# HumaticsLAB/SEAM-Match-RCNN

Measured on NVIDIA B200. Metric: pair_scores_per_sec, higher is better.
Workload: dtype f32 (fp16-operand tcgen05 pass nominates candidates, every result re-scored in f32)

## Files before the change

seam-match-rcnn_b200/csrc/score_exact.cuh:

```cuda
#pragma once
#include <type_traits>
#include <climits>
#include <cstdint>
#include <cuda_fp16.h>
#include "exchange.cuh"
#include "fold.cuh"
#include "score_tc.cuh"
#include "sm100_ptx.cuh"
#include "warp_sort.cuh"

namespace seam {
namespace exact {

constexpr float FP16_MAX = 65504.f;
constexpr float EPS_COEFF = 9.9e-4f;
constexpr float TAG_REL_ERR = 8e-6f;

__device__ __forceinline__ float softmax1(float l0, float l1) {
  const float m = fmaxf(l0, l1);
  const float e0 = expf(l0 - m), e1 = expf(l1 - m);
  return e1 / (e0 + e1);
}

struct Slice {
// ... 43 lines not shown
  l1 = ptx::warp_sum_b(p1) + b1;
}

__global__ void __launch_bounds__(256) prep_gallery_kernel(const float* __restrict__ g, int G,
                                                           const float* __restrict__ fold, __half* __restrict__ g16,
                                                           float* __restrict__ cg, float* __restrict__ gstat) {
  const int warp = threadIdx.x >> 5, lane = threadIdx.x & 31;
  const int j = blockIdx.x * 8 + warp;
  if (j >= G) return;
  const Slice x = load_slice(g + (size_t)j * 256, lane);
  const Slice dw = load_slice(fold + Fold::DW, lane);
  const float xs[8] = {x.lo.x, x.lo.y, x.lo.z, x.lo.w, x.hi.x, x.hi.y, x.hi.z, x.hi.w};
  const float ds[8] = {dw.lo.x, dw.lo.y, dw.lo.z, dw.lo.w, dw.hi.x, dw.hi.y, dw.hi.z, dw.hi.w};
  float c = 0.f, n2 = 0.f, amax = 0.f;
  __half h[8];
#pragma unroll
  for (int e = 0; e < 8; ++e) {
    c = fmaf(ds[e], xs[e] * xs[e], c);
    n2 = fmaf(xs[e], xs[e], n2);
    amax = fmaxf(amax, fabsf(xs[e]));
    h[e] = __float2half_rn(xs[e]);
  }
  __half* dst = g16 + (size_t)j * 256;
  *reinterpret_cast<uint2*>(dst + 4 * lane) = *reinterpret_cast<const uint2*>(&h[0]);
  *reinterpret_cast<uint2*>(dst + 128 + 4 * lane) = *reinterpret_cast<const uint2*>(&h[4]);
  c = ptx::warp_sum(c);
  n2 = ptx::warp_sum(n2);
  amax = ptx::warp_max(amax);
  if (lane == 0) {
    cg[j] = c;
    atomicMax(reinterpret_cast<unsigned int*>(gstat), __float_as_uint(sqrtf(n2)));
    if (!(amax < FP16_MAX)) atomicMax(reinterpret_cast<unsigned int*>(gstat + 1), __float_as_uint(1.f));
  }
}

__global__ void __launch_bounds__(256) prep_queries_kernel(const float* q, int Q,
                                                           const float* __restrict__ fold, __half* __restrict__ a16,
                                                           float* __restrict__ rq, float* __restrict__ anorm,
                                                           uint32_t* __restrict__ thr_global,
                                                           uint32_t* __restrict__ rowflag,
                                                           int32_t* __restrict__ counters,
                                                           int32_t* __restrict__ xdone, const int x_on,
                                                           const xchg::Exchange xc) {
  const int warp = threadIdx.x >> 5, lane = threadIdx.x & 31;
  const int i = blockIdx.x * 8 + warp;
  if (x_on) {
    const uint32_t step = xchg::current_step(xc);
    xchg::wait_all(xc, xchg::KIND_Q, step);
    q = xc.q_all[xc.rank] + (size_t)(step & 1u) * xc.Q * 256;
  }
  if (blockIdx.x == 0 && threadIdx.x == 0) {
    counters[0] = 0;
    counters[1] = 0;
  }
  if (i >= Q) return;
  const Slice x = load_slice(q + (size_t)i * 256, lane);
  const Slice dw = load_slice(fold + Fold::DW, lane);
  const float xs[8] = {x.lo.x, x.lo.y, x.lo.z, x.lo.w, x.hi.x, x.hi.y, x.hi.z, x.hi.w};
  const float ds[8] = {dw.lo.x, dw.lo.y, dw.lo.z, dw.lo.w, dw.hi.x, dw.hi.y, dw.hi.z, dw.hi.w};
  float r = 0.f, n2 = 0.f, amax = 0.f;
  __half h[8];
#pragma unroll
  for (int e = 0; e < 8; ++e) {
    const float a = -2.f * ds[e] * xs[e];
    r = fmaf(ds[e], xs[e] * xs[e], r);
    n2 = fmaf(a, a, n2);
    amax = fmaxf(amax, fabsf(a));
    h[e] = __float2half_rn(a);
  }
  __half* dst = a16 + (size_t)i * 256;
  *reinterpret_cast<uint2*>(dst + 4 * lane) = *reinterpret_cast<const uint2*>(&h[0]);
  *reinterpret_cast<uint2*>(dst + 128 + 4 * lane) = *reinterpret_cast<const uint2*>(&h[4]);
  r = ptx::warp_sum(r);
  n2 = ptx::warp_sum(n2);
  amax = ptx::warp_max(amax);
  if (lane == 0) {
    rq[i] = r;
    anorm[i] = sqrtf(n2);
    thr_global[i] = ptx::float_to_ordered(-INFINITY);
    rowflag[i] = 0;
    if (xdone) xdone[i] = 0;
    if (!(amax < FP16_MAX)) atomicExch(counters + 1, 1);
  }
}

struct RescoreParams {
  const float* q;
  const float* g;
  const float* fold;
  const uint2* rowbuf;
  const uint32_t* rowcnt;
  const uint32_t* rowflag;
  const uint32_t* thr_global;
  const float* gmax;
  const float* rq;
  const float* anorm;
  const float* gstat;
  int Q, G, nlists, CAP, k, index_offset;
  float* out_score;
  float* out_margin;
  int32_t* out_idx;
  int32_t* counters;
  int32_t* fallback_rows;
  int x_on;
  xchg::Exchange x;
  score::TilePlan plan;
};

struct TopkDest {
  float* score;
  float* margin;
  int32_t* idx;
};
__device__ __forceinline__ TopkDest topk_dest(int x_on, const xchg::Exchange& x, uint32_t step, int qi, int k,
                                              float* out_score, float* out_margin, int32_t* out_idx) {
  TopkDest d;
  if (!x_on) {
    const size_t o = (size_t)qi * k;
    d.score = out_score + o;
    d.margin = out_margin + o;
    d.idx = out_idx + o;
  } else {
    const int ow = xchg::owner_of(x, qi);
    const size_t o = ((((size_t)(step & 1u) * x.world + x.rank) * x.own_max) + (size_t)(qi - x.q_lo[ow])) * k;
    d.score = nullptr;
    d.margin = x.list_margin[ow] + o;
    d.idx = x.list_idx[ow] + o;
  }
  return d;
}

constexpr int RS_SUBL = 4;
constexpr int RESCORE_WBUF = 160;

__device__ __forceinline__ void rescore_merge32(const uint2* wb, int begin, int end, float& cv, uint32_t& cidx,
                                                int lane) {
  float v = -INFINITY;
  uint32_t id = 0xffffffffu;
  if (begin + lane < end) {
    const uint2 e = wb[begin + lane];
    v = __uint_as_float(e.x);
    id = e.y;
  }
  const float worst = __shfl_sync(ptx::FULL_MASK, cv, 31);
  if (!(v > worst)) {
    v = -INFINITY;
    id = 0xffffffffu;
  }
  if (!__any_sync(ptx::FULL_MASK, v > -INFINITY)) return;
  wsort::sort32<false>(v, id, lane);
  if (v > cv) {
    cv = v;
    cidx = id;
  }
  wsort::merge32<true>(cv, cidx, lane);
}

__global__ void __launch_bounds__(256) rescore_kernel(const RescoreParams p) {
  __shared__ uint2 wbuf[8][RESCORE_WBUF];
  __shared__ uint4 qbuf[8][64];
  __shared__ uint32_t qcol[8][64];
  const int warp = threadIdx.x >> 5, lane = threadIdx.x & 31;
  const int qi = blockIdx.x * 8 + warp;
  if (qi >= p.Q) return;
  const uint32_t xstep = p.x_on ? xchg::current_step(p.x) : 0u;
  const float* qbase = p.x_on ? p.x.q_all[p.x.rank] + (size_t)(xstep & 1u) * p.x.Q * 256 : p.q;
  const bool overflow = p.counters[1] != 0 || p.gstat[1] != 0.f;
  bool certified = !overflow && p.rowflag[qi] == 0;
  const float tau = ptx::ordered_to_float(p.thr_global[qi]);
  const int nl_valid = min(p.nlists, 4 * score::pieces_of_row(p.plan, qi));
  float cv = -INFINITY;
  uint32_t cidx = 0xffffffffu;
  uint2* wb = wbuf[warp];
  int fill = 0;
  float cut = tau;
  bool cut_strict = false;
  float cut_lo = tau > -INFINITY ? nextafterf(tau, -INFINITY) : -INFINITY;
  {
    const int nval = nl_valid * 16;
    const float* gmp = p.gmax + (size_t)qi * p.nlists * 16;
    auto start_cut = [&](auto nk_tag) {
      constexpr int NK = decltype(nk_tag)::value;
      uint32_t key[NK];
#pragma unroll
      for (int u = 0; u < NK; ++u) {
        const int i = lane + 32 * u;
        key[u] = i < nval ? ptx::float_to_ordered(gmp[i]) : 0u;
      }
      uint32_t lmax = key[0];
#pragma unroll
      for (int j = 1; j < NK; ++j) lmax = max(lmax, key[j]);
      const uint32_t hi = __reduce_max_sync(ptx::FULL_MASK, lmax);
      const uint32_t lo = __reduce_min_sync(ptx::FULL_MASK, lmax);
      uint32_t K = lo;
      if (hi != lo) {
        const int b0 = 31 - __clz(hi ^ lo);
        K = hi & ~((2u << b0) - 1u);
        for (int b = b0; b >= 0 && b > b0 - 8; --b) {
          const uint32_t T = K | (1u << b);
          uint32_t c = 0;
#pragma unroll
          for (int j = 0; j < NK; ++j)
            asm("{\n.reg .pred p;\nsetp.ge.u32 p, %1, %2;\n@p add.u32 %0, %0, 1;\n}\n" : "+r"(c) : "r"(key[j]), "r"(T));
          if (__reduce_add_sync(ptx::FULL_MASK, c) >= 32u) K = T;
        }
      }
      const float tt = ptx::ordered_to_float(K);
      if (K != 0 && tt > cut) {
        cut = tt;
        cut_lo = nextafterf(tt, -INFINITY);
      }
    };
    if (nval <= 128) start_cut(std::integral_constant<int, 4>{});
    else if (nval <= 256) start_cut(std::integral_constant<int, 8>{});
  }
  const int capq = p.CAP / 2;
  const uint4* rowq = reinterpret_cast<const uint4*>(p.rowbuf) + (size_t)qi * p.nlists * capq;
  uint4* qb = qbuf[warp];
  uint32_t* qc = qcol[warp];
  int qfill = 0;
  auto expand = [&](int start, int count) {
    uint4 rec = make_uint4(0u, 0u, 0u, 0u);
    uint32_t col = 0;
    const bool have = lane < count;
    if (have) {
      rec = qb[start + lane];
      col = qc[start + lane];
    }
    const uint32_t wv[4] = {rec.x, rec.y, rec.z, rec.w};
#pragma unroll
    for (int el = 0; el < 4; ++el) {
      const float ev = __uint_as_float(wv[el]);
      const bool pass = have && ev > cut_lo;
      const uint32_t mask = __ballot_sync(ptx::FULL_MASK, pass);
      if (mask == 0u) continue;
      if (pass) wb[fill + __popc(mask & ((1u << lane) - 1u))] = make_uint2(wv[el], col + el);
      fill += __popc(mask);
    }
    if (fill >= 32) {
      __syncwarp();
      while (fill >= 32) {
        rescore_merge32(wb, fill - 32, fill, cv, cidx, lane);
        fill -= 32;
      }
      const float worst = __shfl_sync(ptx::FULL_MASK, cv, 31);
      if (worst > cut || (worst == cut && worst > -INFINITY)) {
        cut = worst;
        cut_strict = true;
        cut_lo = worst;
      }
    }
    __syncwarp();
  };
  for (int l0 = 0; l0 < nl_valid && certified; l0 += 32) {
    const int my_l = l0 + lane;
    uint32_t my_n = my_l < nl_valid ? p.rowcnt[(size_t)qi * p.nlists + my_l] : 0u;
    if (__any_sync(ptx::FULL_MASK, my_n > (uint32_t)capq)) {
      certified = false;
      break;
    }
    const int nl = min(32, nl_valid - l0);
    for (int j0 = 0; j0 < nl; j0 += RS_SUBL) {
      int n4[RS_SUBL];
      int nmax = 0;
#pragma unroll
      for (int u = 0; u < RS_SUBL; ++u) {
        n4[u] = (int)__shfl_sync(ptx::FULL_MASK, my_n, j0 + u);
        nmax = max(nmax, n4[u]);
      }
      const uint4* lp = rowq + (size_t)(l0 + j0) * capq + lane;
      for (int base = 0; base < nmax; base += 32) {
        uint4 e[RS_SUBL];
#pragma unroll
        for (int u = 0; u < RS_SUBL; ++u)
          e[u] = base + lane < n4[u] ? __ldcs(lp + (size_t)u * capq + base)
                                     : make_uint4(0xff800000u, 0xff800000u, 0xff800000u, 0xff800000u);
#pragma unroll
        for (int u = 0; u < RS_SUBL; ++u) {
          const float m = fmaxf(fmaxf(__uint_as_float(e[u].x), __uint_as_float(e[u].y)),
                                fmaxf(__uint_as_float(e[u].z), __uint_as_float(e[u].w)));
          const bool pass = m > cut_lo;
          const uint32_t mask = __ballot_sync(ptx::FULL_MASK, pass);
          if (mask == 0u) continue;
          if (pass) {
            const int pos = qfill + __popc(mask & ((1u << lane) - 1u));
            qb[pos] = e[u];
            qc[pos] = score::quad_first_col(e[u], l0 + j0 + u);
          }
          qfill += __popc(mask);
          if (qfill >= 32) {
            __syncwarp();
            expand(qfill - 32, 32);
            qfill -= 32;
          }
        }
      }
    }
  }
  __syncwarp();
  if (certified && qfill > 0) expand(0, qfill);
  __syncwarp();
  if (certified && fill > 0) rescore_merge32(wb, 0, fill, cv, cidx, lane);
  const bool valid = (int)cidx >= 0;
  const int n_valid = __popc(__ballot_sync(ptx::FULL_MASK, valid));
  if (n_valid < min(32, p.G)) certified = false;
  const float a_k = __shfl_sync(ptx::FULL_MASK, cv, min(p.k, 32) - 1);
  const float amax = ptx::warp_max(valid ? fabsf(cv) : 0.f);
  const float eps = EPS_COEFF * p.anorm[qi] * p.gstat[0] + 1e-5f + TAG_REL_ERR * amax;
  const float cutoff = a_k - 2.f * eps;
  const bool in_S = valid && cv >= cutoff;
  const uint32_t smask = __ballot_sync(ptx::FULL_MASK, in_S);
  if (p.G > 32 && (smask >> 31)) certified = false;
  const int ns = __popc(smask);

  const Slice qs = load_slice(qbase + (size_t)qi * 256, lane);
  const Slice w0 = load_slice(p.fold + Fold::LAST_W, lane);
  const Slice w1 = load_slice(p.fold + Fold::LAST_W + 256, lane);
  const float b0 = p.fold[Fold::CONSTS + 5], b1 = p.fold[Fold::CONSTS + 6];
  float my_l0 = 0.f, my_l1 = 0.f;
  if (certified) {
    for (int c0 = 0; c0 < ns; c0 += 4) {
      Slice gs[4];
#pragma unroll
      for (int u = 0; u < 4; ++u) {
        const int idx = __shfl_sync(ptx::FULL_MASK, (int)cidx, min(c0 + u, ns - 1));
        gs[u] = load_slice(p.g + (size_t)idx * 256, lane);
      }
      float part[8];
#pragma unroll
      for (int u = 0; u < 4; ++u) sqdiff_dot2(qs, gs[u], w0, w1, part[2 * u], part[2 * u + 1]);
      const float tot = ptx::treduce<8>(part, lane);
      const int u_mine = lane - c0;
      const float l0 = __shfl_sync(ptx::FULL_MASK, tot, (2 * u_mine) & 7) + b0;
      const float l1 = __shfl_sync(ptx::FULL_MASK, tot, (2 * u_mine + 1) & 7) + b1;
      if (u_mine >= 0 && u_mine < 4) {
        my_l0 = l0;
        my_l1 = l1;
      }
    }
  }
  float d = in_S ? my_l1 - my_l0 : -INFINITY;
  int id = in_S ? (int)cidx : INT_MAX;
  const float approx_d = cv + p.rq[qi] + p.fold[Fold::CONSTS + 4];
  const bool violated = in_S && !(fabsf(d - approx_d) <= eps + 2e-5f * (1.f + fabsf(d)));
  if (__any_sync(ptx::FULL_MASK, violated)) certified = false;
  wsort::sort32_rank2(d, id, lane);
  if (lane < p.k) {
    const TopkDest dst = topk_dest(p.x_on, p.x, xstep, qi, p.k, p.out_score, p.out_margin, p.out_idx);
    const bool ok = id != INT_MAX;
    if (dst.score) dst.score[lane] = ok ? softmax1(0.f, d) : 0.f;
    dst.margin[lane] = d;
    dst.idx[lane] = ok ? id + p.index_offset : -1;
  }
  if (!certified && lane == 0) {
    const int slot = atomicAdd(p.counters, 1);
    p.fallback_rows[slot] = qi;
  }
}

struct ExactParams {
  const float* q;
  const float* g;
  const float* fold;
  int Q, G, k, index_offset;
  const int32_t* count;
  const int32_t* rows;
  float* out_score;
  float* out_margin;
  int32_t* out_idx;
  float* part_d;
  int32_t* part_i;
  int32_t* done;
  int x_on;
  xchg::Exchange x;
};

constexpr int EXACT_MIN_SLICE = 128;

__global__ void __launch_bounds__(256) exact_topk_kernel(const ExactParams p) {
  __shared__ float sd[8][32];
  __shared__ int si[8][32];
  __shared__ int s_last;
  const int warp = threadIdx.x >> 5, lane = threadIdx.x & 31;
  const int nrows = p.count ? *p.count : p.Q;
  const uint32_t xstep = p.x_on ? xchg::current_step(p.x) : 0u;
  const float* qbase = p.x_on ? p.x.q_all[p.x.rank] + (size_t)(xstep & 1u) * p.x.Q * 256 : p.q;
  int S = 1;
  if (p.part_d && nrows > 0 && nrows < (int)gridDim.x) S = max(1, min((int)gridDim.x / nrows, p.G / EXACT_MIN_SLICE));
  const long long units = (long long)nrows * S;
  if (units == 0) {
    if (p.x_on) xchg::signal_all(p.x, xchg::KIND_L, xstep, false);
    return;
  }
  const Slice w0 = load_slice(p.fold + Fold::LAST_W, lane);
  const Slice w1 = load_slice(p.fold + Fold::LAST_W + 256, lane);
  const float b0 = p.fold[Fold::CONSTS + 5], b1 = p.fold[Fold::CONSTS + 6];
  float cd;
  int cidx;
  auto cta_merge = [&]() {
    sd[warp][lane] = cd;
    si[warp][lane] = cidx;
    __syncthreads();
    if (warp == 0) {
      float dummy = 0.f;
      for (int w = 1; w < 8; ++w) {
        const float od = sd[w][31 - lane];
        const int oi = si[w][31 - lane];
        if (wsort::ranks_before(od, oi, cd, cidx)) {
          cd = od;
// ... 544 lines not shown
```

seam-match-rcnn_b200/csrc/seam_b200.cu:

```cuda
#include <cmath>
#include <cstdarg>
#include <cstdio>
#include <cstdlib>
#include <cstring>
#include <new>
#include <vector>

#include <cuda.h>
#include <cuda_fp16.h>
#include <cuda_runtime.h>

#include "../../include/seam_b200.h"
#include "aggregate_fused.cuh"
#include "backward.cuh"
#include "fold.cuh"
#include "nlb_gemm.cuh"
#include "score_exact.cuh"
#include "score_tc.cuh"
#include "tower_tc.cuh"

using namespace seam;

typedef CUresult (*PFN_encodeTiled)(CUtensorMap*, CUtensorMapDataType, cuuint32_t, void*, const cuuint64_t*,
                                    const cuuint64_t*, const cuuint32_t*, const cuuint32_t*, CUtensorMapInterleave,
                                    CUtensorMapSwizzle, CUtensorMapL2promotion, CUtensorMapFloatOOBfill);

struct seam_handle {
  int device = 0;
  int num_sms = 0;
  float* fold = nullptr;
  bool have_scorer = false;
  bool have_aggregator = false;
  PFN_encodeTiled encode = nullptr;
  uint64_t launches = 0;
  bool profiling = false;
  unsigned int* watchdog = nullptr;
  __half* tw_conv[4] = {nullptr, nullptr, nullptr, nullptr};
  float* tw_misc = nullptr;
  bool have_tower = false;
  struct Span { int kernel; cudaEvent_t a, b; };
  std::vector<Span> spans;
  std::vector<cudaEvent_t> free_events;
  char err[512] = {0};
};

struct ProfileScope {
  seam_handle* h;
  cudaStream_t stream;
  cudaEvent_t a = nullptr, b = nullptr;
  int kernel;
  static cudaEvent_t get(seam_handle* h) {
    cudaEvent_t e = nullptr;
    if (!h->free_events.empty()) { e = h->free_events.back(); h->free_events.pop_back(); }
    else cudaEventCreate(&e);
    return e;
  }
  ProfileScope(seam_handle* h_, int kernel_, cudaStream_t s) : h(h_), stream(s), kernel(kernel_) {
    if (h->profiling && h->spans.size() < 65536) {
      a = get(h); b = get(h);
      cudaEventRecord(a, stream);
    }
  }
  ~ProfileScope() {
    if (a) {
      cudaEventRecord(b, stream);
      h->spans.push_back({kernel, a, b});
    }
  }
};

static thread_local char g_create_err[256] = "";

static unsigned int* g_watchdog_host[64] = {};

static int fail(seam_handle* h, int code, const char* fmt, ...) {
  va_list ap;
  va_start(ap, fmt);
  if (h) vsnprintf(h->err, sizeof(h->err), fmt, ap);
  else vsnprintf(g_create_err, sizeof(g_create_err), fmt, ap);
  va_end(ap);
  return code;
}
// ... 107 lines not shown
  for (int r = 0; r < x->world; ++r) {
    if (x->q_lo[r + 1] < x->q_lo[r] || x->q_lo[r + 1] - x->q_lo[r] > x->own_max)
      return fail(h, SEAM_ERR_BAD_ARG, "%s: q_lo not monotone or ownership above own_max", who);
    if (!x->q_all[r] || !x->list_margin[r] || !x->list_idx[r] || !x->flags[r])
      return fail(h, SEAM_ERR_BAD_ARG, "%s: null buffer for rank %d", who, r);
    if (have_final && (!x->final_score[r] || !x->final_margin[r] || !x->final_idx[r]))
      return fail(h, SEAM_ERR_BAD_ARG, "%s: final buffers must be given for all ranks or none", who);
    e->q_all[r] = x->q_all[r];
    e->list_margin[r] = x->list_margin[r];
    e->list_idx[r] = x->list_idx[r];
    e->final_score[r] = have_final ? x->final_score[r] : nullptr;
    e->final_margin[r] = have_final ? x->final_margin[r] : nullptr;
    e->final_idx[r] = have_final ? x->final_idx[r] : nullptr;
    e->flags[r] = x->flags[r];
  }
  e->step = x->step;
  e->done = x->done;
  e->q_all_mc = x->world > 1 ? x->q_all_mc : nullptr;
  const bool final_mc = x->world > 1 && have_final && x->final_score_mc && x->final_margin_mc && x->final_idx_mc;
  e->final_score_mc = final_mc ? x->final_score_mc : nullptr;
  e->final_margin_mc = final_mc ? x->final_margin_mc : nullptr;
  e->final_idx_mc = final_mc ? x->final_idx_mc : nullptr;
  return SEAM_OK;
}

__global__ void device_stamp_kernel(uint64_t* dst) { *dst = ptx::globaltimer_ns(); }

extern "C" {

int seam_abi_version(void) { return 3; }

size_t seam_exchange_sizeof(void) { return sizeof(seam_exchange); }

int seam_create(seam_handle** out, int device) {
  if (!out) return fail(nullptr, SEAM_ERR_BAD_ARG, "seam_create: out is null");
  *out = nullptr;
  int ndev = 0;
  cudaError_t e = cudaGetDeviceCount(&ndev);
  if (e != cudaSuccess || ndev == 0)
    return fail(nullptr, SEAM_ERR_CUDA, "no CUDA device available (%s); this library has no CPU path",
                e != cudaSuccess ? cudaGetErrorString(e) : "device count is 0");
  if (device < 0 || device >= ndev) return fail(nullptr, SEAM_ERR_BAD_ARG, "device %d out of range", device);
  cudaDeviceProp prop;
  if ((e = cudaGetDeviceProperties(&prop, device)) != cudaSuccess)
    return fail(nullptr, SEAM_ERR_CUDA, "cudaGetDeviceProperties: %s", cudaGetErrorString(e));
  if (prop.major != 10)
    return fail(nullptr, SEAM_ERR_UNSUPPORTED, "device %d is sm_%d%d; this library is built for sm_100a only", device,
                prop.major, prop.minor);
  seam_handle* h = new (std::nothrow) seam_handle();
  if (!h) return fail(nullptr, SEAM_ERR_CUDA, "out of host memory");
  h->device = device;
  h->num_sms = prop.multiProcessorCount;
  DeviceGuard guard(device);
  if ((e = cudaMalloc(&h->fold, sizeof(float) * Fold::TOTAL)) != cudaSuccess) {
    delete h;
    return fail(nullptr, SEAM_ERR_CUDA, "cudaMalloc(fold): %s", cudaGetErrorString(e));
  }
  cudaMemset(h->fold, 0, sizeof(float) * Fold::TOTAL);
  void* fn = nullptr;
  cudaDriverEntryPointQueryResult qres;
  e = cudaGetDriverEntryPoint("cuTensorMapEncodeTiled", &fn, cudaEnableDefault, &qres);
  if (e != cudaSuccess || qres != cudaDriverEntryPointSuccess || !fn) {
    cudaFree(h->fold);
    delete h;
    return fail(nullptr, SEAM_ERR_CUDA, "cuTensorMapEncodeTiled not available from the driver");
  }
  h->encode = reinterpret_cast<PFN_encodeTiled>(fn);
  if (device < 64) {
    if (!g_watchdog_host[device]) {
      unsigned int* hp = nullptr;
      if (cudaHostAlloc(reinterpret_cast<void**>(&hp), 1024, cudaHostAllocMapped) == cudaSuccess) {
        memset(hp, 0, 1024);
        unsigned int* dptr = nullptr;
        if (cudaHostGetDevicePointer(reinterpret_cast<void**>(&dptr), hp, 0) == cudaSuccess &&
            cudaMemcpyToSymbol(ptx::g_watchdog, &dptr, sizeof(dptr)) == cudaSuccess)
          g_watchdog_host[device] = hp;
      }
      cudaGetLastError();
    }
    h->watchdog = g_watchdog_host[device];
  }
  cudaFuncSetAttribute(score::score_topk_kernel<0>, cudaFuncAttributeMaxDynamicSharedMemorySize,
                       (int)score::SMEM_BYTES);
  cudaFuncSetAttribute(score::score_topk_kernel<score::VAR_RANK>, cudaFuncAttributeMaxDynamicSharedMemorySize,
                       (int)score::SMEM_BYTES);
  opt_in_aggregate_smem<float>();
  opt_in_aggregate_smem<__half>();
  cudaFuncSetAttribute(bwd::agg_backward_kernel, cudaFuncAttributeMaxDynamicSharedMemorySize,
                       (int)bwd::agg_bwd_smem_bytes(bwd::BWD_MAX_T));
  cudaFuncSetAttribute(tower::conv3x3_kernel, cudaFuncAttributeMaxDynamicSharedMemorySize, (int)tower::SMEM_BYTES);
  cudaFuncSetAttribute(nlbgemm::nlb_full_front_kernel, cudaFuncAttributeMaxDynamicSharedMemorySize,
                       (int)((SEAM_MAX_T * 257 + 2 * SEAM_MAX_T) * sizeof(float)));
  if ((e = cudaGetLastError()) != cudaSuccess) {
    cudaFree(h->fold);
    delete h;
    return fail(nullptr, SEAM_ERR_CUDA, "cudaFuncSetAttribute: %s", cudaGetErrorString(e));
  }
  *out = h;
  return SEAM_OK;
}

void seam_destroy(seam_handle* h) {
  if (!h) return;
  {
    DeviceGuard guard(h->device);
    for (auto& sp : h->spans) { cudaEventDestroy(sp.a); cudaEventDestroy(sp.b); }
// ... 512 lines not shown
    const size_t n = (size_t)Q * k;
    fill_empty_topk_kernel<<<(unsigned)((n + 255) / 256), 256, 0, stream>>>(out_score, out_margin, out_idx, n);
    SEAM_LAUNCHED(h, "fill_empty_topk_kernel");
    return SEAM_OK;
  }
  ScoreWorkspace w;
  int rc = carve_score_workspace(h, "seam_score_topk", false, q, Q, g, g16, cg, gstat, G, workspace, workspace_bytes, &w);
  if (rc != SEAM_OK) return rc;

  {
    ProfileScope prof(h, SEAM_KERNEL_PREP_QUERIES, stream);
    exact::prep_queries_kernel<<<(Q + 7) / 8, 256, 0, stream>>>(q, Q, h->fold, w.a16, w.rq, w.anorm, w.thr, w.rowflag,
                                                                w.counters, w.xdone, x_on, xe);
    SEAM_LAUNCHED(h, "prep_queries_kernel");
  }

  CUtensorMap tmA, tmB;
  score::Params sp;
  if ((rc = score_kernel_args(h, w, Q, g16, cg, G, &tmA, &tmB, &sp)) != SEAM_OK) return rc;
  {
    ProfileScope prof(h, SEAM_KERNEL_SCORE, stream);
    score::score_topk_kernel<0><<<w.plan.tiles.nb, score::THREADS, score::SMEM_BYTES, stream>>>(tmA, tmB, sp);
    SEAM_LAUNCHED(h, "score_topk_kernel");
  }

  exact::RescoreParams rp;
  rp.q = q;
  rp.g = g;
  rp.fold = h->fold;
  rp.rowbuf = w.rowbuf;
  rp.rowcnt = w.rowcnt;
  rp.rowflag = w.rowflag;
  rp.thr_global = w.thr;
  rp.gmax = w.gmax;
  rp.rq = w.rq;
  rp.anorm = w.anorm;
  rp.gstat = gstat;
  rp.Q = Q;
  rp.G = G;
  rp.nlists = w.plan.P * score::NQ;
  rp.CAP = w.plan.CAP;
  rp.k = k;
  rp.index_offset = index_offset;
  rp.out_score = out_score;
  rp.out_margin = out_margin;
  rp.out_idx = out_idx;
  rp.counters = w.counters;
  rp.fallback_rows = w.frows;
  rp.x_on = x_on;
  rp.x = xe;
  rp.plan = w.plan.tiles;
  {
    ProfileScope prof(h, SEAM_KERNEL_RESCORE, stream);
    exact::rescore_kernel<<<(Q + 7) / 8, 256, 0, stream>>>(rp);
    SEAM_LAUNCHED(h, "rescore_kernel");
  }

  exact::ExactParams ep;
  ep.q = q;
  ep.g = g;
  ep.fold = h->fold;
  ep.Q = Q;
  ep.G = G;
  ep.k = k;
  ep.index_offset = index_offset;
  ep.count = w.counters;
  ep.rows = w.frows;
  ep.out_score = out_score;
  ep.out_margin = out_margin;
  ep.out_idx = out_idx;
  ep.part_d = w.xpart_d;
  ep.part_i = w.xpart_i;
  ep.done = w.xdone;
  ep.x_on = x_on;
  ep.x = xe;
  {
    ProfileScope prof(h, SEAM_KERNEL_EXACT, stream);
    exact::exact_topk_kernel<<<2 * h->num_sms, 256, 0, stream>>>(ep);
    SEAM_LAUNCHED(h, "exact_topk_kernel");
  }
  if (stats) SEAM_CUDA(h, cudaMemcpyAsync(stats, w.counters, 4, cudaMemcpyDeviceToDevice, stream));
  return SEAM_OK;
}

int seam_score_topk(seam_handle* h, const float* q, int Q, const float* g, const void* g16, const float* cg,
                    const float* gstat, int G, int index_offset, int k, float* out_score, float* out_margin,
                    int32_t* out_idx, int32_t* stats, void* workspace, size_t workspace_bytes, void* stream_) {
  if (!h) return SEAM_ERR_BAD_ARG;
  return score_topk_impl(h, nullptr, q, Q, g, g16, cg, gstat, G, index_offset, k, out_score, out_margin, out_idx, stats,
                         workspace, workspace_bytes, stream_);
}

static int search_impl(seam_handle* h, const void* seq, bool f16, const uint8_t* mask, const int32_t* lens, int Tmax,
                       int Q, int64_t frame_stride, int64_t track_stride, float* q_out, const float* g, const void* g16,
                       const float* cg, const float* gstat, int G, int index_offset, int k, float* out_score,
                       float* out_margin, int32_t* out_idx, int32_t* stats, void* workspace, size_t workspace_bytes,
                       void* stream_, const char* who) {
  if (!h) return SEAM_ERR_BAD_ARG;
  if (!q_out && Q > 0) return fail(h, SEAM_ERR_BAD_ARG, "%s: q_out is null", who);
  int rc = aggregate_impl(h, nullptr, 0, 0, seq, f16, mask, lens, Tmax, Q, frame_stride, track_stride, q_out, nullptr,
                          static_cast<cudaStream_t>(stream_), who);
  if (rc != SEAM_OK) return rc;
  return score_topk_impl(h, nullptr, q_out, Q, g, g16, cg, gstat, G, index_offset, k, out_score, out_margin, out_idx, stats,
                         workspace, workspace_bytes, stream_);
}

int seam_search(seam_handle* h, const float* seq, const uint8_t* mask, const int32_t* lens, int Tmax, int Q,
// ... 401 lines not shown
```

seam-match-rcnn_b200/csrc/sm100_ptx.cuh:

```cuda
#pragma once
#include <cstdint>
#include <cuda.h>
#include <cuda_runtime.h>

namespace seam {
namespace ptx {

constexpr uint32_t FULL_MASK = 0xffffffffu;

__device__ __forceinline__ uint32_t smem_u32(const void* p) {
  return static_cast<uint32_t>(__cvta_generic_to_shared(p));
}

__device__ __forceinline__ uint64_t globaltimer_ns() {
  uint64_t t;
  asm volatile("mov.u64 %0, %%globaltimer;" : "=l"(t));
  return t;
}

__device__ __forceinline__ void mbar_init(uint64_t* bar, uint32_t count) {
  asm volatile("mbarrier.init.shared::cta.b64 [%0], %1;" ::"r"(smem_u32(bar)), "r"(count) : "memory");
}
__device__ __forceinline__ void fence_mbar_init() {
  asm volatile("fence.mbarrier_init.release.cluster;" ::: "memory");
// ... 84 lines not shown
      "selp.u32 %0, 1, 0, p;\n"
      "}\n"
      : "=r"(pred));
  return pred != 0;
}

__device__ __forceinline__ void mbar_wait_idle(uint64_t* bar, uint32_t parity, uint32_t sleep_ns, uint32_t tag = 0) {
  uint64_t t0 = 0;
  while (!mbar_try_wait(bar, parity)) {
    __nanosleep(sleep_ns);
    const uint64_t now = globaltimer_ns();
    if (t0 == 0) t0 = now;
    else if (now - t0 > 2000000000ull) watchdog_trap(tag, smem_u32(bar), parity);
  }
}

__device__ __forceinline__ void fence_proxy_async_smem() {
  asm volatile("fence.proxy.async.shared::cta;" ::: "memory");
}

__device__ __forceinline__ void prefetch_tensormap(const CUtensorMap* m) {
  asm volatile("prefetch.tensormap [%0];" ::"l"(reinterpret_cast<uint64_t>(m)) : "memory");
}
__device__ __forceinline__ void tma_load_2d(void* smem_dst, const CUtensorMap* m, uint64_t* bar, int c0, int c1) {
  asm volatile(
      "cp.async.bulk.tensor.2d.shared::cluster.global.mbarrier::complete_tx::bytes [%0], [%1, {%3, %4}], [%2];"
      ::"r"(smem_u32(smem_dst)), "l"(reinterpret_cast<uint64_t>(m)), "r"(smem_u32(bar)), "r"(c0), "r"(c1)
      : "memory");
}
__device__ __forceinline__ void tma_load_3d_hint(void* smem_dst, const CUtensorMap* m, uint64_t* bar, int c0, int c1, int c2,
                                                 uint64_t policy) {
  asm volatile(
      "cp.async.bulk.tensor.3d.shared::cluster.global.mbarrier::complete_tx::bytes.L2::cache_hint [%0], [%1, {%3, %4, %5}], [%2], %6;"
      ::"r"(smem_u32(smem_dst)), "l"(reinterpret_cast<uint64_t>(m)), "r"(smem_u32(bar)), "r"(c0), "r"(c1), "r"(c2), "l"(policy)
      : "memory");
}
__device__ __forceinline__ void bulk_load_1d(void* smem_dst, const void* gsrc, uint32_t bytes, uint64_t* bar) {
  asm volatile(
      "cp.async.bulk.shared::cluster.global.mbarrier::complete_tx::bytes [%0], [%1], %2, [%3];"
      ::"r"(smem_u32(smem_dst)), "l"(reinterpret_cast<uint64_t>(gsrc)), "r"(bytes), "r"(smem_u32(bar))
      : "memory");
}

__device__ __forceinline__ void bulk_store_1d(void* gdst, const void* smem_src, uint32_t bytes) {
  asm volatile("cp.async.bulk.global.shared::cta.bulk_group [%0], [%1], %2;" ::"l"(reinterpret_cast<uint64_t>(gdst)),
               "r"(smem_u32(smem_src)), "r"(bytes)
               : "memory");
}
__device__ __forceinline__ void bulk_commit() { asm volatile("cp.async.bulk.commit_group;" ::: "memory"); }
__device__ __forceinline__ void bulk_wait_read() { asm volatile("cp.async.bulk.wait_group.read 0;" ::: "memory"); }
__device__ __forceinline__ void bulk_wait_all() { asm volatile("cp.async.bulk.wait_group 0;" ::: "memory"); }
__device__ __forceinline__ void fence_proxy_async_all() { asm volatile("fence.proxy.async;" ::: "memory"); }

__device__ __forceinline__ void tmem_alloc(uint32_t* smem_dst, uint32_t ncols) {
  asm volatile("tcgen05.alloc.cta_group::1.sync.aligned.shared::cta.b32 [%0], %1;" ::"r"(smem_u32(smem_dst)),
               "r"(ncols)
               : "memory");
}
__device__ __forceinline__ void tmem_relinquish() {
  asm volatile("tcgen05.relinquish_alloc_permit.cta_group::1.sync.aligned;" ::: "memory");
}
__device__ __forceinline__ void tmem_dealloc(uint32_t taddr, uint32_t ncols) {
  asm volatile("tcgen05.dealloc.cta_group::1.sync.aligned.b32 %0, %1;" ::"r"(taddr), "r"(ncols) : "memory");
}
__device__ __forceinline__ void tc_fence_before() { asm volatile("tcgen05.fence::before_thread_sync;" ::: "memory"); }
__device__ __forceinline__ void tc_fence_after() { asm volatile("tcgen05.fence::after_thread_sync;" ::: "memory"); }

__device__ __forceinline__ void umma_f16(uint32_t tmem_d, uint64_t adesc, uint64_t bdesc, uint32_t idesc,
                                         uint32_t accumulate) {
  asm volatile(
      "{\n"
      ".reg .pred p;\n"
      "setp.ne.b32 p, %4, 0;\n"
      "tcgen05.mma.cta_group::1.kind::f16 [%0], %1, %2, %3, p;\n"
      "}\n" ::"r"(tmem_d),
      "l"(adesc), "l"(bdesc), "r"(idesc), "r"(accumulate)
      : "memory");
}
__device__ __forceinline__ void umma_tf32(uint32_t tmem_d, uint64_t adesc, uint64_t bdesc, uint32_t idesc,
                                          uint32_t accumulate) {
  asm volatile(
      "{\n"
      ".reg .pred p;\n"
      "setp.ne.b32 p, %4, 0;\n"
      "tcgen05.mma.cta_group::1.kind::tf32 [%0], %1, %2, %3, p;\n"
      "}\n" ::"r"(tmem_d),
      "l"(adesc), "l"(bdesc), "r"(idesc), "r"(accumulate)
      : "memory");
}
__device__ __forceinline__ void umma_f16_ts(uint32_t tmem_d, uint32_t tmem_a, uint64_t bdesc, uint32_t idesc,
                                            uint32_t accumulate) {
  asm volatile(
      "{\n"
      ".reg .pred p;\n"
      "setp.ne.b32 p, %4, 0;\n"
      "tcgen05.mma.cta_group::1.kind::f16 [%0], [%1], %2, %3, p;\n"
      "}\n" ::"r"(tmem_d),
      "r"(tmem_a), "l"(bdesc), "r"(idesc), "r"(accumulate)
      : "memory");
}
__device__ __forceinline__ void umma_commit(uint64_t* bar) {
  asm volatile("tcgen05.commit.cta_group::1.mbarrier::arrive::one.shared::cluster.b64 [%0];" ::"r"(smem_u32(bar))
               : "memory");
}

__device__ __forceinline__ uint64_t umma_desc_k_sw128(uint32_t smem_addr) {
// ... 155 lines not shown
```

Before: 1039 billion.

## Make rescore kernel persistent with atomic row claiming and cp.async prefetch

Converts rescore_kernel into a persistent kernel sized to occupancy. Each warp claims its next query row through an atomic counter and prefetches that row's header, list counts and gmax into shared memory with cp.async while it finishes the current row. The fold last-layer weights are also loaded once per CTA into shared memory. The aim is to hide per-row global load latency and cut launch and tail overhead, at the cost of extra shared memory, an atomic per row, and more complex control flow.

```diff
diff --git a/seam-match-rcnn_b200/csrc/score_exact.cuh b/seam-match-rcnn_b200/csrc/score_exact.cuh
--- a/seam-match-rcnn_b200/csrc/score_exact.cuh
+++ b/seam-match-rcnn_b200/csrc/score_exact.cuh
@@ -119,6 +119,7 @@
   if (blockIdx.x == 0 && threadIdx.x == 0) {
     counters[0] = 0;
     counters[1] = 0;
+    counters[2] = 0;
   }
   if (i >= Q) return;
   const Slice x = load_slice(q + (size_t)i * 256, lane);
@@ -199,6 +200,7 @@
 
 constexpr int RS_SUBL = 4;
 constexpr int RESCORE_WBUF = 160;
+constexpr int RS_THREADS = 256;
 
 __device__ __forceinline__ void rescore_merge32(const uint2* wb, int begin, int end, float& cv, uint32_t& cidx,
                                                 int lane) {
@@ -223,205 +225,261 @@
   wsort::merge32<true>(cv, cidx, lane);
 }
 
-__global__ void __launch_bounds__(256) rescore_kernel(const RescoreParams p) {
+struct RescoreRowStage {
+  uint32_t hdr[4];
+  int row, nl_valid;
+  uint32_t cnt[32];
+  float4 gmax[64];
+};
+enum { RS_HDR_FLAG, RS_HDR_THR, RS_HDR_RQ, RS_HDR_ANORM };
+
+__device__ __forceinline__ void rescore_stage_row(const RescoreParams& p, int qi, RescoreRowStage& st, int lane) {
+  const int nl_valid = min(p.nlists, 4 * score::pieces_of_row(p.plan, qi));
+  if (lane == 0) {
+    st.row = qi;
+    st.nl_valid = nl_valid;
+  }
+  if (lane < 4) {
+    const void* src = lane == RS_HDR_FLAG ? (const void*)(p.rowflag + qi)
+                    : lane == RS_HDR_THR  ? (const void*)(p.thr_global + qi)
+                    : lane == RS_HDR_RQ   ? (const void*)(p.rq + qi)
+                                          : (const void*)(p.anorm + qi);
+    ptx::cp_async_4(&st.hdr[lane], src);
+  }
+  if (lane < nl_valid) ptx::cp_async_4(&st.cnt[lane], p.rowcnt + (size_t)qi * p.nlists + lane);
+  const int nchunk = nl_valid * 4;
+  if (nchunk <= 64) {
+    const float4* src = reinterpret_cast<const float4*>(p.gmax + (size_t)qi * p.nlists * 16);
+    if (lane < nchunk) ptx::cp_async_16(&st.gmax[lane], src + lane);
+    if (lane + 32 < nchunk) ptx::cp_async_16(&st.gmax[lane + 32], src + lane + 32);
+  }
+}
+
+__global__ void __launch_bounds__(RS_THREADS) rescore_kernel(const RescoreParams p) {
   __shared__ uint2 wbuf[8][RESCORE_WBUF];
   __shared__ uint4 qbuf[8][64];
   __shared__ uint32_t qcol[8][64];
+  __shared__ RescoreRowStage stage[8];
+  __shared__ float4 wlast[2][64];
+  __shared__ uint32_t s_xstep;
+  __shared__ int s_overflow;
   const int warp = threadIdx.x >> 5, lane = threadIdx.x & 31;
-  const int qi = blockIdx.x * 8 + warp;
-  if (qi >= p.Q) return;
-  const uint32_t xstep = p.x_on ? xchg::current_step(p.x) : 0u;
-  const float* qbase = p.x_on ? p.x.q_all[p.x.rank] + (size_t)(xstep & 1u) * p.x.Q * 256 : p.q;
-  const bool overflow = p.counters[1] != 0 || p.gstat[1] != 0.f;
-  bool certified = !overflow && p.rowflag[qi] == 0;
-  const float tau = ptx::ordered_to_float(p.thr_global[qi]);
-  const int nl_valid = min(p.nlists, 4 * score::pieces_of_row(p.plan, qi));
-  float cv = -INFINITY;
-  uint32_t cidx = 0xffffffffu;
-  uint2* wb = wbuf[warp];
-  int fill = 0;
-  float cut = tau;
-  bool cut_strict = false;
-  float cut_lo = tau > -INFINITY ? nextafterf(tau, -INFINITY) : -INFINITY;
-  {
-    const int nval = nl_valid * 16;
-    const float* gmp = p.gmax + (size_t)qi * p.nlists * 16;
-    auto start_cut = [&](auto nk_tag) {
-      constexpr int NK = decltype(nk_tag)::value;
-      uint32_t key[NK];
-#pragma unroll
-      for (int u = 0; u < NK; ++u) {
-        const int i = lane + 32 * u;
-        key[u] = i < nval ? ptx::float_to_ordered(gmp[i]) : 0u;
-      }
-      uint32_t lmax = key[0];
-#pragma unroll
-      for (int j = 1; j < NK; ++j) lmax = max(lmax, key[j]);
-      const uint32_t hi = __reduce_max_sync(ptx::FULL_MASK, lmax);
-      const uint32_t lo = __reduce_min_sync(ptx::FULL_MASK, lmax);
-      uint32_t K = lo;
-      if (hi != lo) {
-        const int b0 = 31 - __clz(hi ^ lo);
-        K = hi & ~((2u << b0) - 1u);
-        for (int b = b0; b >= 0 && b > b0 - 8; --b) {
-          const uint32_t T = K | (1u << b);
-          uint32_t c = 0;
-#pragma unroll
-          for (int j = 0; j < NK; ++j)
-            asm("{\n.reg .pred p;\nsetp.ge.u32 p, %1, %2;\n@p add.u32 %0, %0, 1;\n}\n" : "+r"(c) : "r"(key[j]), "r"(T));
-          if (__reduce_add_sync(ptx::FULL_MASK, c) >= 32u) K = T;
-        }
-      }
-      const float tt = ptx::ordered_to_float(K);
-      if (K != 0 && tt > cut) {
-        cut = tt;
-        cut_lo = nextafterf(tt, -INFINITY);
-      }
+  for (int i = threadIdx.x; i < 128; i += RS_THREADS)
+    wlast[i >> 6][i & 63] = reinterpret_cast<const float4*>(p.fold + Fold::LAST_W)[i];
+  if (threadIdx.x == 0) {
+    s_xstep = p.x_on ? xchg::current_step(p.x) : 0u;
+    s_overflow = p.counters[1] != 0 || p.gstat[1] != 0.f;
+  }
+  __syncthreads();
+  const int first = blockIdx.x * 8 + warp;
+  if (first >= p.Q) return;
+  rescore_stage_row(p, first, stage[warp], lane);
+  while (true) {
+    const int lane = ptx::thread_index() & 31, warp = ptx::thread_index() >> 5;
+    RescoreRowStage& st = stage[warp];
+    uint2* wb = wbuf[warp];
+    uint4* qb = qbuf[warp];
+    uint32_t* qc = qcol[warp];
+    const int capq = p.CAP / 2;
+    int claim = 0;
+    if (lane == 0) claim = atomicAdd(p.counters + 2, 1);
+    ptx::cp_async_wait_all();
+    __syncwarp();
+    const int qi = st.row, nl_valid = st.nl_valid;
+    if (qi >= p.Q) break;
+    bool certified = !s_overflow && st.hdr[RS_HDR_FLAG] == 0;
+    const float tau = ptx::ordered_to_float(st.hdr[RS_HDR_THR]);
+    float cv = -INFINITY;
+    uint32_t cidx = 0xffffffffu;
+    int fill = 0;
+    float cut = tau;
+    bool cut_strict = false;
+    float cut_lo = tau > -INFINITY ? nextafterf(tau, -INFINITY) : -INFINITY;
+    {
+      const int nval = nl_valid * 16;
+      const float* gmp = reinterpret_cast<const float*>(st.gmax);
+      auto start_cut = [&](auto nk_tag) {
+        constexpr int NK = decltype(nk_tag)::value;
+        uint32_t key[NK];
+#pragma unroll
+        for (int u = 0; u < NK; ++u) {
+          const int i = lane + 32 * u;
+          key[u] = i < nval ? ptx::float_to_ordered(gmp[i]) : 0u;
+        }
+        uint32_t lmax = key[0];
+#pragma unroll
+        for (int j = 1; j < NK; ++j) lmax = max(lmax, key[j]);
+        const uint32_t hi = __reduce_max_sync(ptx::FULL_MASK, lmax);
+        const uint32_t lo = __reduce_min_sync(ptx::FULL_MASK, lmax);
+        uint32_t K = lo;
+        if (hi != lo) {
+          const int b0 = 31 - __clz(hi ^ lo);
+          K = hi & ~((2u << b0) - 1u);
+          for (int b = b0; b >= 0 && b > b0 - 8; --b) {
+            const uint32_t T = K | (1u << b);
+            uint32_t c = 0;
+#pragma unroll
+            for (int j = 0; j < NK; ++j)
+              asm("{\n.reg .pred p;\nsetp.ge.u32 p, %1, %2;\n@p add.u32 %0, %0, 1;\n}\n" : "+r"(c) : "r"(key[j]), "r"(T));
+            if (__reduce_add_sync(ptx::FULL_MASK, c) >= 32u) K = T;
+          }
+        }
+        const float tt = ptx::ordered_to_float(K);
+        if (K != 0 && tt > cut) {
+          cut = tt;
+          cut_lo = nextafterf(tt, -INFINITY);
+        }
+      };
+      if (nval <= 128) start_cut(std::integral_constant<int, 4>{});
+      else if (nval <= 256) start_cut(std::integral_constant<int, 8>{});
+    }
+    const uint4* rowq = reinterpret_cast<const uint4*>(p.rowbuf) + (size_t)qi * p.nlists * capq;
+    int qfill = 0;
+    auto expand = [&](int start, int count) {
+      uint4 rec = make_uint4(0u, 0u, 0u, 0u);
+      uint32_t col = 0;
+      const bool have = lane < count;
+      if (have) {
+        rec = qb[start + lane];
+        col = qc[start + lane];
+      }
+      const uint32_t wv[4] = {rec.x, rec.y, rec.z, rec.w};
+#pragma unroll
+      for (int el = 0; el < 4; ++el) {
+        const float ev = __uint_as_float(wv[el]);
+        const bool pass = have && ev > cut_lo;
+        const uint32_t mask = __ballot_sync(ptx::FULL_MASK, pass);
+        if (mask == 0u) continue;
+        if (pass) wb[fill + __popc(mask & ((1u << lane) - 1u))] = make_uint2(wv[el], col + el);
+        fill += __popc(mask);
+      }
+      if (fill >= 32) {
+        __syncwarp();
+        while (fill >= 32) {
+          rescore_merge32(wb, fill - 32, fill, cv, cidx, lane);
+          fill -= 32;
+        }
+        const float worst = __shfl_sync(ptx::FULL_MASK, cv, 31);
+        if (worst > cut || (worst == cut && worst > -INFINITY)) {
+          cut = worst;
+          cut_strict = true;
+          cut_lo = worst;
+        }
+      }
+      __syncwarp();
     };
-    if (nval <= 128) start_cut(std::integral_constant<int, 4>{});
-    else if (nval <= 256) start_cut(std::integral_constant<int, 8>{});
-  }
-  const int capq = p.CAP / 2;
-  const uint4* rowq = reinterpret_cast<const uint4*>(p.rowbuf) + (size_t)qi * p.nlists * capq;
-  uint4* qb = qbuf[warp];
-  uint32_t* qc = qcol[warp];
-  int qfill = 0;
-  auto expand = [&](int start, int count) {
-    uint4 rec = make_uint4(0u, 0u, 0u, 0u);
-    uint32_t col = 0;
-    const bool have = lane < count;
-    if (have) {
-      rec = qb[start + lane];
-      col = qc[start + lane];
-    }
-    const uint32_t wv[4] = {rec.x, rec.y, rec.z, rec.w};
-#pragma unroll
-    for (int el = 0; el < 4; ++el) {
-      const float ev = __uint_as_float(wv[el]);
-      const bool pass = have && ev > cut_lo;
-      const uint32_t mask = __ballot_sync(ptx::FULL_MASK, pass);
-      if (mask == 0u) continue;
-      if (pass) wb[fill + __popc(mask & ((1u << lane) - 1u))] = make_uint2(wv[el], col + el);
-      fill += __popc(mask);
-    }
-    if (fill >= 32) {
-      __syncwarp();
-      while (fill >= 32) {
-        rescore_merge32(wb, fill - 32, fill, cv, cidx, lane);
-        fill -= 32;
-      }
-      const float worst = __shfl_sync(ptx::FULL_MASK, cv, 31);
-      if (worst > cut || (worst == cut && worst > -INFINITY)) {
-        cut = worst;
-        cut_strict = true;
-        cut_lo = worst;
+    for (int l0 = 0; l0 < nl_valid && certified; l0 += 32) {
+      const int my_l = l0 + lane;
+      uint32_t my_n = 0u;
+      if (my_l < nl_valid) my_n = l0 == 0 ? st.cnt[lane] : p.rowcnt[(size_t)qi * p.nlists + my_l];
+      if (__any_sync(ptx::FULL_MASK, my_n > (uint32_t)capq)) {
+        certified = false;
+        break;
+      }
+      const int nl = min(32, nl_valid - l0);
+      for (int j0 = 0; j0 < nl; j0 += RS_SUBL) {
+        int n4[RS_SUBL];
+        int nmax = 0;
+#pragma unroll
+        for (int u = 0; u < RS_SUBL; ++u) {
+          n4[u] = (int)__shfl_sync(ptx::FULL_MASK, my_n, j0 + u);
+          nmax = max(nmax, n4[u]);
+        }
+        const uint4* lp = rowq + (size_t)(l0 + j0) * capq + lane;
+        for (int base = 0; base < nmax; base += 32) {
+          uint4 e[RS_SUBL];
+#pragma unroll
+          for (int u = 0; u < RS_SUBL; ++u)
+            e[u] = base + lane < n4[u] ? __ldcs(lp + (size_t)u * capq + base)
+                                       : make_uint4(0xff800000u, 0xff800000u, 0xff800000u, 0xff800000u);
+#pragma unroll
+          for (int u = 0; u < RS_SUBL; ++u) {
+            const float m = fmaxf(fmaxf(__uint_as_float(e[u].x), __uint_as_float(e[u].y)),
+                                  fmaxf(__uint_as_float(e[u].z), __uint_as_float(e[u].w)));
+            const bool pass = m > cut_lo;
+            const uint32_t mask = __ballot_sync(ptx::FULL_MASK, pass);
+            if (mask == 0u) continue;
+            if (pass) {
+              const int pos = qfill + __popc(mask & ((1u << lane) - 1u));
+              qb[pos] = e[u];
+              qc[pos] = score::quad_first_col(e[u], l0 + j0 + u);
+            }
+            qfill += __popc(mask);
+            if (qfill >= 32) {
+              __syncwarp();
+              expand(qfill - 32, 32);
+              qfill -= 32;
+            }
+          }
+        }
       }
     }
     __syncwarp();
-  };
-  for (int l0 = 0; l0 < nl_valid && certified; l0 += 32) {
-    const int my_l = l0 + lane;
-    uint32_t my_n = my_l < nl_valid ? p.rowcnt[(size_t)qi * p.nlists + my_l] : 0u;
-    if (__any_sync(ptx::FULL_MASK, my_n > (uint32_t)capq)) {
-      certified = false;
-      break;
-    }
-    const int nl = min(32, nl_valid - l0);
-    for (int j0 = 0; j0 < nl; j0 += RS_SUBL) {
-      int n4[RS_SUBL];
-      int nmax = 0;
-#pragma unroll
-      for (int u = 0; u < RS_SUBL; ++u) {
-        n4[u] = (int)__shfl_sync(ptx::FULL_MASK, my_n, j0 + u);
-        nmax = max(nmax, n4[u]);
-      }
-      const uint4* lp = rowq + (size_t)(l0 + j0) * capq + lane;
-      for (int base = 0; base < nmax; base += 32) {
-        uint4 e[RS_SUBL];
-#pragma unroll
-        for (int u = 0; u < RS_SUBL; ++u)
-          e[u] = base + lane < n4[u] ? __ldcs(lp + (size_t)u * capq + base)
-                                     : make_uint4(0xff800000u, 0xff800000u, 0xff800000u, 0xff800000u);
-#pragma unroll
-        for (int u = 0; u < RS_SUBL; ++u) {
-          const float m = fmaxf(fmaxf(__uint_as_float(e[u].x), __uint_as_float(e[u].y)),
-                                fmaxf(__uint_as_float(e[u].z), __uint_as_float(e[u].w)));
-          const bool pass = m > cut_lo;
-          const uint32_t mask = __ballot_sync(ptx::FULL_MASK, pass);
-          if (mask == 0u) continue;
-          if (pass) {
-            const int pos = qfill + __popc(mask & ((1u << lane) - 1u));
-            qb[pos] = e[u];
-            qc[pos] = score::quad_first_col(e[u], l0 + j0 + u);
-          }
-          qfill += __popc(mask);
-          if (qfill >= 32) {
-            __syncwarp();
-            expand(qfill - 32, 32);
-            qfill -= 32;
-          }
-        }
-      }
-    }
-  }
-  __syncwarp();
-  if (certified && qfill > 0) expand(0, qfill);
-  __syncwarp();
-  if (certified && fill > 0) rescore_merge32(wb, 0, fill, cv, cidx, lane);
-  const bool valid = (int)cidx >= 0;
-  const int n_valid = __popc(__ballot_sync(ptx::FULL_MASK, valid));
-  if (n_valid < min(32, p.G)) certified = false;
-  const float a_k = __shfl_sync(ptx::FULL_MASK, cv, min(p.k, 32) - 1);
-  const float amax = ptx::warp_max(valid ? fabsf(cv) : 0.f);
-  const float eps = EPS_COEFF * p.anorm[qi] * p.gstat[0] + 1e-5f + TAG_REL_ERR * amax;
-  const float cutoff = a_k - 2.f * eps;
-  const bool in_S = valid && cv >= cutoff;
-  const uint32_t smask = __ballot_sync(ptx::FULL_MASK, in_S);
-  if (p.G > 32 && (smask >> 31)) certified = false;
-  const int ns = __popc(smask);
-
-  const Slice qs = load_slice(qbase + (size_t)qi * 256, lane);
-  const Slice w0 = load_slice(p.fold + Fold::LAST_W, lane);
-  const Slice w1 = load_slice(p.fold + Fold::LAST_W + 256, lane);
-  const float b0 = p.fold[Fold::CONSTS + 5], b1 = p.fold[Fold::CONSTS + 6];
-  float my_l0 = 0.f, my_l1 = 0.f;
-  if (certified) {
-    for (int c0 = 0; c0 < ns; c0 += 4) {
-      Slice gs[4];
-#pragma unroll
-      for (int u = 0; u < 4; ++u) {
-        const int idx = __shfl_sync(ptx::FULL_MASK, (int)cidx, min(c0 + u, ns - 1));
-        gs[u] = load_slice(p.g + (size_t)idx * 256, lane);
-      }
-      float part[8];
-#pragma unroll
-      for (int u = 0; u < 4; ++u) sqdiff_dot2(qs, gs[u], w0, w1, part[2 * u], part[2 * u + 1]);
-      const float tot = ptx::treduce<8>(part, lane);
-      const int u_mine = lane - c0;
-      const float l0 = __shfl_sync(ptx::FULL_MASK, tot, (2 * u_mine) & 7) + b0;
-      const float l1 = __shfl_sync(ptx::FULL_MASK, tot, (2 * u_mine + 1) & 7) + b1;
-      if (u_mine >= 0 && u_mine < 4) {
-        my_l0 = l0;
-        my_l1 = l1;
-      }
-    }
-  }
-  float d = in_S ? my_l1 - my_l0 : -INFINITY;
-  int id = in_S ? (int)cidx : INT_MAX;
-  const float approx_d = cv + p.rq[qi] + p.fold[Fold::CONSTS + 4];
-  const bool violated = in_S && !(fabsf(d - approx_d) <= eps + 2e-5f * (1.f + fabsf(d)));
-  if (__any_sync(ptx::FULL_MASK, violated)) certified = false;
-  wsort::sort32_rank2(d, id, lane);
-  if (lane < p.k) {
-    const TopkDest dst = topk_dest(p.x_on, p.x, xstep, qi, p.k, p.out_score, p.out_margin, p.out_idx);
-    const bool ok = id != INT_MAX;
-    if (dst.score) dst.score[lane] = ok ? softmax1(0.f, d) : 0.f;
-    dst.margin[lane] = d;
-    dst.idx[lane] = ok ? id + p.index_offset : -1;
-  }
-  if (!certified && lane == 0) {
-    const int slot = atomicAdd(p.counters, 1);
-    p.fallback_rows[slot] = qi;
+    if (certified && qfill > 0) expand(0, qfill);
+    __syncwarp();
+    if (certified && fill > 0) rescore_merge32(wb, 0, fill, cv, cidx, lane);
+    const bool valid = (int)cidx >= 0;
+    const int n_valid = __popc(__ballot_sync(ptx::FULL_MASK, valid));
+    if (n_valid < min(32, p.G)) certified = false;
+    const float a_k = __shfl_sync(ptx::FULL_MASK, cv, min(p.k, 32) - 1);
+    const float amax = ptx::warp_max(valid ? fabsf(cv) : 0.f);
+    const float eps = EPS_COEFF * __uint_as_float(st.hdr[RS_HDR_ANORM]) * p.gstat[0] + 1e-5f + TAG_REL_ERR * amax;
+    const float cutoff = a_k - 2.f * eps;
+    const bool in_S = valid && cv >= cutoff;
+    const uint32_t smask = __ballot_sync(ptx::FULL_MASK, in_S);
+    if (p.G > 32 && (smask >> 31)) certified = false;
+    const int ns = __popc(smask);
+    const float approx_d = cv + __uint_as_float(st.hdr[RS_HDR_RQ]) + p.fold[Fold::CONSTS + 4];
+
+    const int next = gridDim.x * 8 + __shfl_sync(ptx::FULL_MASK, claim, 0);
+    __syncwarp();
+    if (next < p.Q) rescore_stage_row(p, next, st, lane);
+    else if (lane == 0) st.row = next;
+
+    const float* qbase = p.x_on ? p.x.q_all[p.x.rank] + (size_t)(s_xstep & 1u) * p.x.Q * 256 : p.q;
+    const Slice qs = load_slice(qbase + (size_t)qi * 256, lane);
+    const Slice w0 = {wlast[0][lane], wlast[0][32 + lane]};
+    const Slice w1 = {wlast[1][lane], wlast[1][32 + lane]};
+    float my_l0 = 0.f, my_l1 = 0.f;
+    if (certified) {
+      for (int c0 = 0; c0 < ns; c0 += 4) {
+        Slice gs[4];
+#pragma unroll
+        for (int u = 0; u < 4; ++u) {
+          const int idx = __shfl_sync(ptx::FULL_MASK, (int)cidx, min(c0 + u, ns - 1));
+          gs[u] = load_slice(p.g + (size_t)idx * 256, lane);
+        }
+        float part[8];
+#pragma unroll
+        for (int u = 0; u < 4; ++u) sqdiff_dot2(qs, gs[u], w0, w1, part[2 * u], part[2 * u + 1]);
+        const float tot = ptx::treduce<8>(part, lane);
+        const int u_mine = lane - c0;
+        const float l0 = __shfl_sync(ptx::FULL_MASK, tot, (2 * u_mine) & 7);
+        const float l1 = __shfl_sync(ptx::FULL_MASK, tot, (2 * u_mine + 1) & 7);
+        if (u_mine >= 0 && u_mine < 4) {
+          my_l0 = l0;
+          my_l1 = l1;
+        }
+      }
+      my_l0 += p.fold[Fold::CONSTS + 5];
+      my_l1 += p.fold[Fold::CONSTS + 6];
+    }
+    float d = in_S ? my_l1 - my_l0 : -INFINITY;
+    int id = in_S ? (int)cidx : INT_MAX;
+    const bool violated = in_S && !(fabsf(d - approx_d) <= eps + 2e-5f * (1.f + fabsf(d)));
+    if (__any_sync(ptx::FULL_MASK, violated)) certified = false;
+    wsort::sort32_rank2(d, id, lane);
+    if (lane < p.k) {
+      const TopkDest dst = topk_dest(p.x_on, p.x, s_xstep, qi, p.k, p.out_score, p.out_margin, p.out_idx);
+      const bool ok = id != INT_MAX;
+      if (dst.score) dst.score[lane] = ok ? softmax1(0.f, d) : 0.f;
+      dst.margin[lane] = d;
+      dst.idx[lane] = ok ? id + p.index_offset : -1;
+    }
+    if (!certified && lane == 0) {
+      const int slot = atomicAdd(p.counters, 1);
+      p.fallback_rows[slot] = qi;
+    }
   }
 }
 
diff --git a/seam-match-rcnn_b200/csrc/seam_b200.cu b/seam-match-rcnn_b200/csrc/seam_b200.cu
--- a/seam-match-rcnn_b200/csrc/seam_b200.cu
+++ b/seam-match-rcnn_b200/csrc/seam_b200.cu
@@ -28,6 +28,7 @@
 struct seam_handle {
   int device = 0;
   int num_sms = 0;
+  int rescore_ctas = 0;
   float* fold = nullptr;
   bool have_scorer = false;
   bool have_aggregator = false;
@@ -241,6 +242,14 @@
   h->device = device;
   h->num_sms = prop.multiProcessorCount;
   DeviceGuard guard(device);
+  int rescore_per_sm = 0;
+  if ((e = cudaOccupancyMaxActiveBlocksPerMultiprocessor(&rescore_per_sm, exact::rescore_kernel, exact::RS_THREADS, 0)) !=
+      cudaSuccess || rescore_per_sm < 1) {
+    delete h;
+    return fail(nullptr, SEAM_ERR_CUDA, "rescore_kernel occupancy: %s",
+                e != cudaSuccess ? cudaGetErrorString(e) : "no CTA fits an SM");
+  }
+  h->rescore_ctas = rescore_per_sm * h->num_sms;
   if ((e = cudaMalloc(&h->fold, sizeof(float) * Fold::TOTAL)) != cudaSuccess) {
     delete h;
     return fail(nullptr, SEAM_ERR_CUDA, "cudaMalloc(fold): %s", cudaGetErrorString(e));
@@ -859,7 +868,8 @@
   rp.plan = w.plan.tiles;
   {
     ProfileScope prof(h, SEAM_KERNEL_RESCORE, stream);
-    exact::rescore_kernel<<<(Q + 7) / 8, 256, 0, stream>>>(rp);
+    const int rows_ctas = (Q + 7) / 8;
+    exact::rescore_kernel<<<rows_ctas < h->rescore_ctas ? rows_ctas : h->rescore_ctas, exact::RS_THREADS, 0, stream>>>(rp);
     SEAM_LAUNCHED(h, "rescore_kernel");
   }
 
diff --git a/seam-match-rcnn_b200/csrc/sm100_ptx.cuh b/seam-match-rcnn_b200/csrc/sm100_ptx.cuh
--- a/seam-match-rcnn_b200/csrc/sm100_ptx.cuh
+++ b/seam-match-rcnn_b200/csrc/sm100_ptx.cuh
@@ -160,6 +160,19 @@
 __device__ __forceinline__ void bulk_wait_all() { asm volatile("cp.async.bulk.wait_group 0;" ::: "memory"); }
 __device__ __forceinline__ void fence_proxy_async_all() { asm volatile("fence.proxy.async;" ::: "memory"); }
 
+__device__ __forceinline__ int thread_index() {
+  int r;
+  asm volatile("mov.u32 %0, %%tid.x;" : "=r"(r));
+  return r;
+}
+__device__ __forceinline__ void cp_async_4(void* smem_dst, const void* gsrc) {
+  asm volatile("cp.async.ca.shared.global [%0], [%1], 4;" ::"r"(smem_u32(smem_dst)), "l"(gsrc) : "memory");
+}
+__device__ __forceinline__ void cp_async_16(void* smem_dst, const void* gsrc) {
+  asm volatile("cp.async.cg.shared.global [%0], [%1], 16;" ::"r"(smem_u32(smem_dst)), "l"(gsrc) : "memory");
+}
+__device__ __forceinline__ void cp_async_wait_all() { asm volatile("cp.async.wait_all;" ::: "memory"); }
+
 __device__ __forceinline__ void tmem_alloc(uint32_t* smem_dst, uint32_t ncols) {
   asm volatile("tcgen05.alloc.cta_group::1.sync.aligned.shared::cta.b32 [%0], %1;" ::"r"(smem_u32(smem_dst)),
                "r"(ncols)
```

Result: no change. 1040 billion (median of 6 runs) (+0.1%).
